# willSapgreen/structure-from-motion

Measured on AMD Instinct MI355X. Metric: BA LM-iterations/sec + final reprojection RMSE, 50 cams x 20k pts, higher is better.
Workload: dtype f64; 1 GPU; C3: 50 cams x 20000 pts/rank @ 60% visibility, lambda=5, Schur BA; observations_per_rank=599866, points_total=20000, parallelism=single GPU, collective_backend=none (plain python, no process group), collective=allreduce, schur=auto

## Files before the change

structure-from-motion_amd/csrc/sfm_ba.h:

```cpp
#pragma once

#include <utility>
#include <vector>

#include "sfm_common.h"

namespace sfm {

constexpr int kSchurCB = 18;
constexpr int kSchurRB = 128;
constexpr int kSchurMaxChunks = 128;
constexpr int kSchurKSL = 16;
constexpr int kInvRowsMaxNbk = 52;
constexpr size_t kRowsLdsBudget = 156 * 1024;
constexpr int kLinGridPerCu = 3;

constexpr int kStatSlots = 256;
constexpr int kNB = 32;
constexpr int kBlk = kNB * kNB;
__host__ __device__ inline size_t red_blk_base(int br, int bc) { return ((size_t)br * (br + 1) / 2 + bc) * kBlk; }
__host__ __device__ inline int red_blk_off(int i, int k) { return i * kNB + k; }
__host__ __device__ inline int red_lblk_off(int i, int k) { return (k >> 3) * 256 + (k & 3) * 64 + i * 2 + ((k >> 2) & 1); }
__host__ __device__ inline size_t red_index(int row, int col) {
  return red_blk_base(row >> 5, col >> 5) + red_blk_off(row & 31, col & 31);
}
__host__ __device__ inline size_t red_rhs_off(int nbk) { return (size_t)nbk * (nbk + 1) / 2 * kBlk; }
__host__ __device__ inline size_t red_size(int nbk) { return red_rhs_off(nbk) + (size_t)nbk * kNB; }

struct BaDev {
  int V = 0, N = 0;
  long long M = 0;
  int P = 0;
  int nbk = 0;
  int* pt_ptr = nullptr;
  int* cam_idx = nullptr;
  int* obs_pt = nullptr;
  double* u = nullptr;
  double* v = nullptr;
  double* cams = nullptr;
  double* px = nullptr;
  double* py = nullptr;
  double* pz = nullptr;
  CamPrep* prep[2] = {nullptr, nullptr};
  double* Z = nullptr;
  double* Zd = nullptr;
  int zp = 0;
  int zrows = 0;
  double* lin_ws = nullptr;
  double* red = nullptr;
  double* delta = nullptr;
  double* ldiag = nullptr;
  double* xinv = nullptr;
  int* sync_ctr = nullptr;
  unsigned* flow = nullptr;
  const void* flow_tasks = nullptr;
  int flow_ntasks = 0;
  int debug = 0;
  int* status = nullptr;
  int* sinfo = nullptr;
  double* cost = nullptr;
  double* cost_ws = nullptr;
  int* iter_count = nullptr;
  unsigned long long* stamps = nullptr;
};

__device__ __forceinline__ void cost_reduce(const BaDev& d, int nrows) {
  double s = 0;
  for (int r = threadIdx.x; r < nrows; r += 64) s += d.cost_ws[r];
  s = wave_sum(s);
  if (threadIdx.x == 0) d.cost[min(*d.iter_count, kStatSlots - 1)] = s;
}

__device__ __forceinline__ void cam_reduce_slice(const BaDev& d, int nrows, int t, int slice, int nslices) {
  if (t >= d.V * 35) return;
  const int per = (nrows + nslices - 1) / nslices;
  const int r0 = slice * per, r1 = min(nrows, r0 + per);
  double s = 0;
  for (int r = r0; r < r1; ++r) s += d.lin_ws[(size_t)r * d.V * 35 + t];
  if (s == 0.0) return;
  const int c = t / 35, e = t % 35;
// ... 78 lines not shown
  ~PhaseEvents() { for (hipEvent_t x : ev) (void)hipEventDestroy(x); }
  int mark(hipStream_t s) {
    if (!timed) return SFM_OK;
    hipEvent_t x;
    SFM_HIP(hipEventCreate(&x));
    ev.push_back(x);
    SFM_HIP(hipEventRecord(x, s));
    return SFM_OK;
  }
  int marks() const { return (int)ev.size(); }
  float elapsed_ms(int i) const {
    float t = 0.f;
    if (i < 0 || i + 1 >= marks() || hipEventElapsedTime(&t, ev[i], ev[i + 1]) != hipSuccess) return 0.f;
    return t;
  }
  const bool timed;
  std::vector<hipEvent_t> ev;
};

constexpr unsigned kBaMagic = 0x5F3BA001u;

struct BaScene {
  BaDev dev;
  double* own_red = nullptr;
  int max_track = 0;
  int cur = 0;
  bool prep_valid = false;
  int lin_rows = 0;
  int lin_grid = 0;
  bool red_clean = false;
  bool backsub_pending = false;
  double pending_lambda = 0;
  int pending_quirks = 0;
  bool last_reduce_deferred = false;
  bool reduce_deferred = false;
  void* schur_ws = nullptr;
  int* schur_blk_ptr = nullptr;
  bool schur_mfma_ok = false;
  const void* flow_tasks_red = nullptr;
  int flow_ntasks_red = 0;
  double* flow_camsum = nullptr;
  bool cam_list_built = false;
  int* cam_ptr = nullptr;
  int* cam_obs = nullptr;
  std::vector<int> h_cam_ptr;
  bool rows_built = false, rows_ok = false;
  void* cam_ent = nullptr;
  unsigned long long* cam_pairs = nullptr;
  std::vector<unsigned long long> h_cam_pairs;
  void* rows_table = nullptr;
  int* rows_first = nullptr;
  void* rows_ws = nullptr;
  int rows_R = 0, rows_tpr = 0, rows_wgs = 0, rows_groups = 0;
  int rows_tpl = 0, rows_cp = 7;
  std::vector<void*> owned;
};

int scene_alloc_bytes(BaScene& sc, void** ptr, size_t bytes);
template <typename T>
int scene_alloc(BaScene& sc, T*& ptr, size_t count) {
  void* q = nullptr;
  SFM_TRY(scene_alloc_bytes(sc, &q, sizeof(T) * count));
  ptr = static_cast<T*>(q);
  return SFM_OK;
}

// ... 74 lines not shown
```

structure-from-motion_amd/csrc/sfm_ba.hip:

```cpp
#include <algorithm>
#include <vector>

#include "sfm_ba.h"
#include "sfm_ba_terms.h"

namespace sfm {

__global__ void ba_cam_prep_kernel(int V, const double* __restrict__ cams, CamPrep* __restrict__ prep,
                                   int* __restrict__ status) {
  const int c = blockIdx.x * blockDim.x + threadIdx.x;
  if (c >= V) return;
  CamPrep out;
  const int st = cam_prepare(cams + 7 * c, &out);
  prep[c] = out;
  report_status(status, st, c);
}

template <int G, int LDS_MODE, bool DENSE_Z, bool FUSED, int THREADS = 256, int LOSS = SFM_LOSS_NONE>
__global__ __launch_bounds__(THREADS) void ba_linearize_kernel(BaDev d, int cur, double lambda, int quirks, LossArg<LOSS> la) {
  static_assert(!FUSED || LDS_MODE == 2, "the fused kernel keeps both camera sets in LDS");
  extern __shared__ double lds[];
  unsigned long long* stamp = (d.stamps && blockIdx.x == 0 && threadIdx.x == 0) ? d.stamps + 192 : nullptr;
  int sidx = 0;
  if (stamp) stamp[sidx++] = __builtin_amdgcn_s_memtime();
  constexpr bool PREP_LDS = LDS_MODE == 2, ACC_LDS = LDS_MODE >= 1;
  double* lds_prep = lds;
  double* lds_acc = lds + (PREP_LDS ? (size_t)d.V * 19 : 0);
  double* lds_old = lds + (size_t)d.V * (19 + 35);
  double* lds_delta = lds_old + (size_t)d.V * 19;
  const CamPrep* gprep = d.prep[cur];
  if (ACC_LDS) {
    if (PREP_LDS) {
      const double* src = reinterpret_cast<const double*>(gprep);
      for (int i = threadIdx.x; i < d.V * 19; i += blockDim.x) lds_prep[i] = src[i];
    }
    if (FUSED) {
      const double* src = reinterpret_cast<const double*>(d.prep[cur ^ 1]);
      for (int i = threadIdx.x; i < d.V * 19; i += blockDim.x) lds_old[i] = src[i];
      for (int i = threadIdx.x; i < d.V * 7; i += blockDim.x) lds_delta[i] = d.delta[i];
    }
    for (int i = threadIdx.x; i < d.V * 35; i += blockDim.x) lds_acc[i] = 0.0;
    __syncthreads();
  }
  if (FUSED) {
    const size_t n_red = red_size(d.nbk);
    for (size_t i = (size_t)blockIdx.x * blockDim.x + threadIdx.x; i < n_red; i += (size_t)gridDim.x * blockDim.x) d.red[i] = 0.0;
  }
  if (stamp) stamp[sidx++] = __builtin_amdgcn_s_memtime();
  constexpr int GPB = THREADS / G;
  const int lane_g = threadIdx.x % G;
  const int grp = threadIdx.x / G;
  double* S = d.red;
  double* rhs = d.red + red_rhs_off(d.nbk);
  double cost = 0.0;

  for (int p0 = blockIdx.x * GPB; p0 < d.N; p0 += gridDim.x * GPB) {
    const int p = p0 + grp;
    int beg = 0, end = 0;
    double X = 0, Y = 0, Z = 0;
    if (p < d.N) {
      beg = d.pt_ptr[p]; end = d.pt_ptr[p + 1];
      X = d.px[p]; Y = d.py[p]; Z = d.pz[p];
    }
    const bool single = (end - beg) <= G;
    double r[2], Jp[14], Jx[6];
    double rho = 0;
    int cam = 0;
    double uo = 0, vo = 0;
    const int o1 = beg + lane_g;
    if (single && o1 < end) { cam = d.cam_idx[o1]; uo = d.u[o1]; vo = d.v[o1]; }
    if (FUSED) {
      double a[9] = {0, 0, 0, 0, 0, 0, 0, 0, 0};
      for (int o = o1; o < end; o += G) {
        if (!single) { cam = d.cam_idx[o]; uo = d.u[o]; vo = d.v[o]; }
        CamPrep c;
        load_cam(c, reinterpret_cast<const CamPrep*>(lds_old) + cam);
        obs_terms_loss<LOSS>(c, X, Y, Z, uo, vo, quirks, la, r, Jp, Jx, rho);
        const double* dp = lds_delta + 7 * cam;
        double e0 = r[0], e1 = r[1];
#pragma unroll
        for (int i = 0; i < 7; ++i) { e0 -= Jp[i] * dp[i]; e1 -= Jp[7 + i] * dp[i]; }
        a[0] += Jx[0] * Jx[0] + Jx[3] * Jx[3];
        a[1] += Jx[1] * Jx[0] + Jx[4] * Jx[3];
        a[2] += Jx[1] * Jx[1] + Jx[4] * Jx[4];
        a[3] += Jx[2] * Jx[0] + Jx[5] * Jx[3];
        a[4] += Jx[2] * Jx[1] + Jx[5] * Jx[4];
        a[5] += Jx[2] * Jx[2] + Jx[5] * Jx[5];
        a[6] += Jx[0] * e0 + Jx[3] * e1;
        a[7] += Jx[1] * e0 + Jx[4] * e1;
        a[8] += Jx[2] * e0 + Jx[5] * e1;
      }
#pragma unroll
      for (int k = 0; k < 9; ++k) a[k] = group_sum<G>(a[k]);
      a[0] += lambda; a[2] += lambda; a[5] += lambda;
      double li[6];
      chol3_inv_fast(a, li);
      const double y0 = li[0] * a[6];
      const double y1 = li[1] * a[6] + li[2] * a[7];
      const double y2 = li[3] * a[6] + li[4] * a[7] + li[5] * a[8];
      X += li[0] * y0 + li[1] * y1 + li[3] * y2;
      Y += li[2] * y1 + li[4] * y2;
      Z += li[5] * y2;
      if (lane_g == 0 && p < d.N) { d.px[p] = X; d.py[p] = Y; d.pz[p] = Z; }
    }
    double v6[6] = {0, 0, 0, 0, 0, 0}, g3[3] = {0, 0, 0};
    for (int o = o1; o < end; o += G) {
      if (!single) { cam = d.cam_idx[o]; uo = d.u[o]; vo = d.v[o]; }
      CamPrep c;
      load_cam(c, PREP_LDS ? reinterpret_cast<const CamPrep*>(lds_prep) + cam : gprep + cam);
      obs_terms_loss<LOSS>(c, X, Y, Z, uo, vo, quirks, la, r, Jp, Jx, rho);
      v6[0] += Jx[0] * Jx[0] + Jx[3] * Jx[3];
      v6[1] += Jx[1] * Jx[0] + Jx[4] * Jx[3];
      v6[2] += Jx[1] * Jx[1] + Jx[4] * Jx[4];
      v6[3] += Jx[2] * Jx[0] + Jx[5] * Jx[3];
      v6[4] += Jx[2] * Jx[1] + Jx[5] * Jx[4];
      v6[5] += Jx[2] * Jx[2] + Jx[5] * Jx[5];
      g3[0] += Jx[0] * r[0] + Jx[3] * r[1];
      g3[1] += Jx[1] * r[0] + Jx[4] * r[1];
      g3[2] += Jx[2] * r[0] + Jx[5] * r[1];
    }
    if (stamp && sidx < 60) { asm volatile("" :: "v"(v6[0])); stamp[sidx++] = __builtin_amdgcn_s_memtime(); }
#pragma unroll
    for (int k = 0; k < 6; ++k) v6[k] = group_sum<G>(v6[k]);
#pragma unroll
    for (int k = 0; k < 3; ++k) g3[k] = group_sum<G>(g3[k]);
    v6[0] += lambda; v6[2] += lambda; v6[5] += lambda;
    double li[6];
    chol3_inv_fast(v6, li);
    const double y0 = li[0] * g3[0];
    const double y1 = li[1] * g3[0] + li[2] * g3[1];
    const double y2 = li[3] * g3[0] + li[4] * g3[1] + li[5] * g3[2];
    const double h2 = li[5] * y2;
    const double h1 = li[2] * y1 + li[4] * y2;
    const double h0 = li[0] * y0 + li[1] * y1 + li[3] * y2;
    if (stamp && sidx < 60) { asm volatile("" :: "v"(h0)); stamp[sidx++] = __builtin_amdgcn_s_memtime(); }
    for (int o = o1; o < end; o += G) {
      if (!single) {
        cam = d.cam_idx[o];
        CamPrep c;
        load_cam(c, PREP_LDS ? reinterpret_cast<const CamPrep*>(lds_prep) + cam : gprep + cam);
        obs_terms_loss<LOSS>(c, X, Y, Z, d.u[o], d.v[o], quirks, la, r, Jp, Jx, rho);
      }
      double acc[35];
      {
        double m0[3], m1[3];
        m0[0] = Jx[0] * li[0];
        m0[1] = Jx[0] * li[1] + Jx[1] * li[2];
        m0[2] = Jx[0] * li[3] + Jx[1] * li[4] + Jx[2] * li[5];
        m1[0] = Jx[3] * li[0];
        m1[1] = Jx[3] * li[1] + Jx[4] * li[2];
        m1[2] = Jx[3] * li[3] + Jx[4] * li[4] + Jx[5] * li[5];
        if (DENSE_Z) {
          double* zr = d.Zd + (size_t)(3 * p) * d.zp + 7 * cam;
          typedef double d2u __attribute__((ext_vector_type(2), aligned(8)));
#pragma unroll
          for (int j = 0; j < 3; ++j) {
            double zz[7];
#pragma unroll
            for (int i = 0; i < 7; ++i) zz[i] = Jp[i] * m0[j] + Jp[7 + i] * m1[j];
            double* row = zr + (size_t)j * d.zp;
#pragma unroll
            for (int i = 0; i < 6; i += 2) *reinterpret_cast<d2u*>(row + i) = d2u{zz[i], zz[i + 1]};
            row[6] = zz[6];
          }
        } else {
          double* zo = d.Z + (size_t)o * 21;
          typedef double d2u __attribute__((ext_vector_type(2), aligned(8)));
// ... 27 lines not shown
        for (int i = 0; i < 7; ++i) {
#pragma unroll
          for (int j = 0; j <= i; ++j) { acc[k] = Jp[i] * Jp[j] + Jp[7 + i] * Jp[7 + j]; ++k; }
          acc[28 + i] = Jp[i] * e0 + Jp[7 + i] * e1;
        }
        k = 0;
        for (int i = 0; i < 7; ++i)
          for (int j = 0; j <= i; ++j) { atomicAdd(&S[red_index(7 * cam + i, 7 * cam + j)], acc[k]); ++k; }
        for (int i = 0; i < 7; ++i) atomicAdd(&rhs[7 * cam + i], acc[28 + i]);
      }
    }
  }
  if (stamp && sidx < 62) stamp[sidx++] = __builtin_amdgcn_s_memtime();
  {
    __shared__ double wcost[THREADS / 64];
    cost = wave_sum(cost);
    if ((threadIdx.x & 63) == 0) wcost[threadIdx.x >> 6] = cost;
    __syncthreads();
    if (threadIdx.x == 0) {
      double t = 0;
#pragma unroll
      for (int w = 0; w < THREADS / 64; ++w) t += wcost[w];
      d.cost_ws[blockIdx.x] = t;
    }
  }
  if (ACC_LDS) {
    __syncthreads();
    double* row = d.lin_ws + (size_t)blockIdx.x * d.V * 35;
    for (int t = threadIdx.x; t < d.V * 35; t += blockDim.x) row[t] = lds_acc[t];
  }
  if (stamp && sidx < 63) { stamp[sidx++] = __builtin_amdgcn_s_memtime(); stamp[63] = sidx; }
}

template <int G, bool CAMS_IN_LDS, int LOSS = SFM_LOSS_NONE>
__global__ __launch_bounds__(256) void ba_backsub_kernel(BaDev d, int cur, double lambda, int quirks, LossArg<LOSS> la) {
  extern __shared__ double lds[];
  double* lds_prep = lds;
  double* lds_delta = lds + (size_t)d.V * 19;
  const CamPrep* gprep = d.prep[cur];
  if (CAMS_IN_LDS) {
    const double* src = reinterpret_cast<const double*>(gprep);
    for (int i = threadIdx.x; i < d.V * 19; i += blockDim.x) lds_prep[i] = src[i];
    for (int i = threadIdx.x; i < d.V * 7; i += blockDim.x) lds_delta[i] = d.delta[i];
    __syncthreads();
  }
  constexpr int GPB = 256 / G;
  const int lane_g = threadIdx.x % G;
  const int grp = threadIdx.x / G;
  {
    const size_t n_red = red_size(d.nbk);
    for (size_t i = (size_t)blockIdx.x * blockDim.x + threadIdx.x; i < n_red; i += (size_t)gridDim.x * blockDim.x) d.red[i] = 0.0;
  }
  for (int p0 = blockIdx.x * GPB; p0 < d.N; p0 += gridDim.x * GPB) {
    const int p = p0 + grp;
    int beg = 0, end = 0;
    double X = 0, Y = 0, Z = 0;
    if (p < d.N) {
      beg = d.pt_ptr[p]; end = d.pt_ptr[p + 1];
      X = d.px[p]; Y = d.py[p]; Z = d.pz[p];
    }
    double a[9] = {0, 0, 0, 0, 0, 0, 0, 0, 0};
    for (int o = beg + lane_g; o < end; o += G) {
      const int cam = d.cam_idx[o];
      CamPrep c;
      load_cam(c, CAMS_IN_LDS ? reinterpret_cast<const CamPrep*>(lds_prep) + cam : gprep + cam);
      double r[2], Jp[14], Jx[6], rho;
      obs_terms_loss<LOSS>(c, X, Y, Z, d.u[o], d.v[o], quirks, la, r, Jp, Jx, rho);
      const double* dp = CAMS_IN_LDS ? lds_delta + 7 * cam : d.delta + 7 * cam;
      double e0 = r[0], e1 = r[1];
#pragma unroll
      for (int i = 0; i < 7; ++i) { e0 -= Jp[i] * dp[i]; e1 -= Jp[7 + i] * dp[i]; }
      a[0] += Jx[0] * Jx[0] + Jx[3] * Jx[3];
      a[1] += Jx[1] * Jx[0] + Jx[4] * Jx[3];
      a[2] += Jx[1] * Jx[1] + Jx[4] * Jx[4];
      a[3] += Jx[2] * Jx[0] + Jx[5] * Jx[3];
      a[4] += Jx[2] * Jx[1] + Jx[5] * Jx[4];
      a[5] += Jx[2] * Jx[2] + Jx[5] * Jx[5];
      a[6] += Jx[0] * e0 + Jx[3] * e1;
      a[7] += Jx[1] * e0 + Jx[4] * e1;
      a[8] += Jx[2] * e0 + Jx[5] * e1;
    }
#pragma unroll
    for (int k = 0; k < 9; ++k) a[k] = group_sum<G>(a[k]);
    if (lane_g == 0 && p < d.N) {
      a[0] += lambda; a[2] += lambda; a[5] += lambda;
      double li[6];
      chol3_inv_fast(a, li);
      const double y0 = li[0] * a[6];
      const double y1 = li[1] * a[6] + li[2] * a[7];
      const double y2 = li[3] * a[6] + li[4] * a[7] + li[5] * a[8];
      d.px[p] = X + (li[0] * y0 + li[1] * y1 + li[3] * y2);
      d.py[p] = Y + (li[2] * y1 + li[4] * y2);
// ... 14 lines not shown
  obs_terms(c, d.px[p], d.py[p], d.pz[p], d.u[o], d.v[o], quirks, r, Jp, Jx);
  r_out[2 * o] = r[0]; r_out[2 * o + 1] = r[1];
  for (int k = 0; k < 14; ++k) Jp_out[14 * o + k] = Jp[k];
  for (int k = 0; k < 6; ++k) Jx_out[6 * o + k] = Jx[k];
}

template <int LOSS>
__global__ void ba_loss_terms_kernel(BaDev d, int cur, int quirks, LossArg<LOSS> la, double* __restrict__ s_out,
                                     double* __restrict__ w_out, double* __restrict__ rho_out) {
  const long long o = blockIdx.x * (long long)blockDim.x + threadIdx.x;
  if (o >= d.M) return;
  const int p = d.obs_pt[o];
  CamPrep c;
  load_cam(c, d.prep[cur] + d.cam_idx[o]);
  double r[2], Jp[14], Jx[6];
  obs_terms(c, d.px[p], d.py[p], d.pz[p], d.u[o], d.v[o], quirks, r, Jp, Jx);
  double s = r[0] * r[0] + r[1] * r[1], w = 1.0, sw = 1.0, rho = s;
  if constexpr (LOSS != SFM_LOSS_NONE) {
    s *= la.inv_d2;
    loss_eval<LOSS>(s, w, sw, rho);
  }
  if (s_out) s_out[o] = s;
  if (w_out) w_out[o] = w;
  if (rho_out) rho_out[o] = rho;
}

static int pick_group(const sfm_ba_problem* p) {
  double mean = p->dev.N > 0 ? (double)p->dev.M / p->dev.N : 1.0;
  int g = 4;
  while (g < 64 && g < mean) g <<= 1;
  return g;
}

template <int LDS, bool WZ, bool FUSED = false>
static void launch_linearize(const sfm_ba_problem* p, int cur, int g, int grid, size_t lds, hipStream_t s, double lambda, int quirks) {
  const BaDev& d = p->dev;
  dispatch_loss(p->loss_kind, [&](auto L) {
    constexpr int LOSS = decltype(L)::value;
    const LossArg<LOSS> la = loss_arg<LOSS>(p);
    dispatch_group<4>(g, [&](auto G) {
      if (p->deterministic)
        ba_linearize_kernel<decltype(G)::value, LDS, WZ, FUSED, 64, LOSS><<<grid, 64, lds, s>>>(d, cur, lambda, quirks, la);
      else
        ba_linearize_kernel<decltype(G)::value, LDS, WZ, FUSED, 256, LOSS><<<grid, 256, lds, s>>>(d, cur, lambda, quirks, la);
    });
  });
}

template <bool LDS>
static void launch_backsub(const sfm_ba_problem* p, int g, int grid, size_t lds, hipStream_t s, double lambda, int quirks) {
  const BaDev& d = p->dev;
  dispatch_loss(p->loss_kind, [&](auto L) {
    constexpr int LOSS = decltype(L)::value;
    const LossArg<LOSS> la = loss_arg<LOSS>(p);
    dispatch_group<4>(g, [&](auto G) {
      ba_backsub_kernel<decltype(G)::value, LDS, LOSS><<<grid, 256, lds, s>>>(d, p->cur, lambda, quirks, la);
    });
  });
}

void ba_tick(sfm_ba_problem* p, int kid, bool begin, hipStream_t s) {
  if (!(p->timing & (1 << kid))) return;
  KernelTimer& t = p->timers[kid];
  if (begin) {
    t.open = (t.calls++ % p->timing_stride) == 0;
    if (!t.open) return;
    if (t.used == (int)t.ev.size()) {
      hipEvent_t a, b;
      (void)hipEventCreate(&a); (void)hipEventCreate(&b);
      t.ev.push_back({a, b});
    }
    (void)hipEventRecord(t.ev[t.used].first, s);
  } else if (t.open) {
    (void)hipEventRecord(t.ev[t.used].second, s);
    t.used++;
    t.open = false;
  }
}

int ba_enqueue_prep(sfm_ba_problem* p) {
  hipStream_t s = p->stream;
  const BaDev& d = p->dev;
  ba_tick(p, SFM_K_PREP, true, s);
  ba_cam_prep_kernel<<<(d.V + 63) / 64, 64, 0, s>>>(d.V, d.cams, d.prep[p->cur], d.status);
  ba_tick(p, SFM_K_PREP, false, s);
  SFM_HIP(hipGetLastError());
  p->prep_valid = true;
  return SFM_OK;
}

bool ba_can_fuse(const sfm_ba_problem* p) {
  return !(p->debug & 16) && sizeof(double) * (size_t)p->dev.V * (19 + 35 + 19 + 7) <= 64 * 1024;
}

static int enqueue_backsub(sfm_ba_problem* p, double lambda, int quirks) {
  hipStream_t s = p->stream;
  const BaDev& d = p->dev;
  const int g = pick_group(p);
  const int gpb = 256 / g;
  int grid = std::min((d.N + gpb - 1) / gpb, 4 * ctx().num_cus);
  if (grid < 1) grid = 1;
  const size_t lds = sizeof(double) * (size_t)d.V * (19 + 7);
  ba_tick(p, SFM_K_BACKSUB, true, s);
  if (lds <= 64 * 1024) launch_backsub<true>(p, g, grid, lds, s, lambda, quirks);
  else launch_backsub<false>(p, g, grid, 0, s, lambda, quirks);
  ba_tick(p, SFM_K_BACKSUB, false, s);
  SFM_HIP(hipGetLastError());
  p->red_clean = true;
  p->cur ^= 1;
  return SFM_OK;
}

int ba_flush(sfm_ba_problem* p) {
  if (!p->backsub_pending) return SFM_OK;
  p->backsub_pending = false;
  return enqueue_backsub(p, p->pending_lambda, p->pending_quirks);
}

int ba_enqueue_linearize_reduce(sfm_ba_problem* p, double lambda, int quirks, bool allow_defer) {
  hipStream_t s = p->stream;
  const BaDev& d = p->dev;
  bool fused = p->backsub_pending && ba_can_fuse(p) && lambda == p->pending_lambda && quirks == p->pending_quirks;
  if (!fused) {
    SFM_TRY(ba_flush(p));
    if (!p->prep_valid) SFM_TRY(ba_enqueue_prep(p));
    if (!p->red_clean) SFM_HIP(hipMemsetAsync(d.red, 0, sizeof(double) * red_size(d.nbk), s));
  }
  p->red_clean = false;
  const int g = pick_group(p);
  const int gpb = (p->deterministic ? 64 : 256) / g;
  int grid = std::min((d.N + gpb - 1) / gpb, kLinGridPerCu * ctx().num_cus);
  if (grid < 1) grid = 1;
  const size_t lds = sizeof(double) * (size_t)d.V * (19 + 35);
  ba_tick(p, SFM_K_LINEARIZE, true, s);
  p->quirks = quirks;
  const bool dense_z = ba_schur_uses_mfma(p);
  if (dense_z) SFM_TRY(ba_schur_prepare_dense(p, s));
  if (!dense_z && d.Z == nullptr && d.M > 0) {
    SFM_TRY(scene_alloc(*p, p->dev.Z, 21 * (size_t)d.M));
  }
  const size_t lds_acc = sizeof(double) * (size_t)d.V * 35;
  const int mode = lds <= 64 * 1024 ? 2 : (lds_acc <= 64 * 1024 ? 1 : 0);
  if (fused) {
    const size_t lds_f = sizeof(double) * (size_t)d.V * (19 + 35 + 19 + 7);
    if (dense_z) launch_linearize<2, true, true>(p, p->cur ^ 1, g, grid, lds_f, s, lambda, quirks);
    else launch_linearize<2, false, true>(p, p->cur ^ 1, g, grid, lds_f, s, lambda, quirks);
    p->backsub_pending = false;
    p->cur ^= 1;
  } else if (mode == 2) {
    if (dense_z) launch_linearize<2, true>(p, p->cur, g, grid, lds, s, lambda, quirks);
    else launch_linearize<2, false>(p, p->cur, g, grid, lds, s, lambda, quirks);
  } else if (mode == 1) {
    if (dense_z) launch_linearize<1, true>(p, p->cur, g, grid, lds_acc, s, lambda, quirks);
    else launch_linearize<1, false>(p, p->cur, g, grid, lds_acc, s, lambda, quirks);
  } else {
    if (dense_z) launch_linearize<0, true>(p, p->cur, g, grid, 0, s, lambda, quirks);
    else launch_linearize<0, false>(p, p->cur, g, grid, 0, s, lambda, quirks);
  }
  p->lin_rows = mode >= 1 ? grid : 0;
  p->lin_grid = grid;
  ba_tick(p, SFM_K_LINEARIZE, false, s);
  SFM_HIP(hipGetLastError());
  SFM_TRY(ba_enqueue_schur(p, s, allow_defer));
  return SFM_OK;
}

int ba_enqueue_solve_update(sfm_ba_problem* p, double lambda, int quirks) {
  hipStream_t s = p->stream;
  SFM_TRY(ba_flush(p));
  ba_tick(p, SFM_K_SOLVE, true, s);
  SFM_TRY(ba_enqueue_reduced_solve(p, lambda));
  ba_tick(p, SFM_K_SOLVE, false, s);
  SFM_HIP(hipGetLastError());
  if (ba_can_fuse(p)) {
    p->backsub_pending = true;
    p->pending_lambda = lambda;
    p->pending_quirks = quirks;
    return SFM_OK;
  }
  return enqueue_backsub(p, lambda, quirks);
}

void ba_graph_drop(sfm_ba_problem* p) {
  for (auto& g : p->body_graph) {
    if (g) (void)hipGraphExecDestroy(g);
    g = nullptr;
  }
}

static int capture_body(sfm_ba_problem* p, double lambda, int quirks) {
  hipStream_t s = p->stream;
  const int slot = p->cur;
  SFM_HIP(hipStreamBeginCapture(s, hipStreamCaptureModeRelaxed));
  int st = ba_enqueue_linearize_reduce(p, lambda, quirks, true);
  if (st == SFM_OK) st = ba_enqueue_solve_update(p, lambda, quirks);
  hipGraph_t graph = nullptr;
  const hipError_t e = hipStreamEndCapture(s, &graph);
  if (st != SFM_OK) { if (graph) (void)hipGraphDestroy(graph); return st; }
  SFM_HIP(e);
  hipGraphExec_t exec = nullptr;
  const hipError_t ei = hipGraphInstantiate(&exec, graph, nullptr, nullptr, 0);
  (void)hipGraphDestroy(graph);
  SFM_HIP(ei);
  p->body_graph[slot] = exec;
  SFM_HIP(hipGraphLaunch(exec, s));
  return SFM_OK;
}

int ba_enqueue_iterations(sfm_ba_problem* p, double lambda, int iters, int quirks) {
  const bool graphs = p->use_graph && p->timing == 0 && p->stream != nullptr && ba_can_fuse(p) && p->comm == nullptr;
  if (graphs && (lambda != p->graph_lambda || quirks != p->graph_quirks)) {
    ba_graph_drop(p);
    p->graph_lambda = lambda;
    p->graph_quirks = quirks;
  }
  for (int it = 0; it < iters; ++it) {
    const bool steady = p->backsub_pending && lambda == p->pending_lambda && quirks == p->pending_quirks;
    if (graphs && steady) {
      if (p->body_graph[p->cur] == nullptr) {
        SFM_TRY(capture_body(p, lambda, quirks));
      } else {
        SFM_HIP(hipGraphLaunch(p->body_graph[p->cur], p->stream));
        p->cur ^= 1;
        p->red_clean = false;
        ++p->graph_replays;
      }
      continue;
    }
    SFM_TRY(ba_enqueue_linearize_reduce(p, lambda, quirks, p->comm == nullptr));
    if (p->comm) SFM_TRY(comm_all_reduce_f64(p->comm, p->dev.red, red_size(p->dev.nbk), p->stream));
    SFM_TRY(ba_enqueue_solve_update(p, lambda, quirks));
  }
  return ba_flush(p);
}

void ba_enqueue_residual_jacobian(sfm_ba_problem* p, int quirks, double* r, double* Jp, double* Jx) {
  const BaDev& d = p->dev;
  ba_residual_jacobian_kernel<<<(unsigned)((d.M + 255) / 256), 256, 0, p->stream>>>(d, p->cur, quirks, d.obs_pt, r, Jp, Jx);
}


void ba_enqueue_loss_terms(sfm_ba_problem* p, int quirks, double* s_out, double* w_out, double* rho_out) {
  const BaDev& d = p->dev;
  const unsigned grid = (unsigned)((d.M + 255) / 256);
  dispatch_loss(p->loss_kind, [&](auto L) {
    constexpr int LOSS = decltype(L)::value;
    ba_loss_terms_kernel<LOSS><<<grid, 256, 0, p->stream>>>(d, p->cur, quirks, loss_arg<LOSS>(p), s_out, w_out, rho_out);
  });
}

}
// ... 1 lines not shown
```

structure-from-motion_amd/csrc/sfm_ba_host.hip:

```cpp
#include <algorithm>
#include <vector>

#include "sfm_ba.h"
#include "sfm_ba_terms.h"
#include "sfm_scan.h"

namespace sfm {

__global__ void ba_structure_kernel(int V, int N, long long M, const int* __restrict__ pt_ptr,
                                    const int* __restrict__ cam_idx, int* __restrict__ obs_pt,
                                    int* __restrict__ blk_ptr, int nblk, int* __restrict__ sinfo) {
  const int p = blockIdx.x * blockDim.x + threadIdx.x;
  if (p >= N) return;
  const int beg = pt_ptr[p], end = pt_ptr[p + 1];
  int* row = blk_ptr + (size_t)p * (nblk + 1);
  if (beg < 0 || end < beg || end > M) {
    report_status(sinfo, 1, p);
    for (int b = 0; b <= nblk; ++b) row[b] = 0;
    return;
  }
  int prev = -1, b = 0;
  for (int o = beg; o < end; ++o) {
    const int c = cam_idx[o];
    if (c < 0 || c >= V) { report_status(sinfo, 2, o); continue; }
// ... 259 lines not shown
  SFM_HIP(hipMemcpyAsync(p->h_cam_ptr.data(), p->cam_ptr, sizeof(int) * ((size_t)V + 1), hipMemcpyDeviceToHost, s));
  SFM_TRY(stream_sync(s));
  p->cam_list_built = true;
  return SFM_OK;
}

int scene_alloc_bytes(BaScene& sc, void** ptr, size_t bytes) {
  const hipError_t e = pool_alloc(ptr, std::max<size_t>(1, bytes));
  if (e != hipSuccess) return hip_fail(e, "hipMalloc of a scene buffer", __LINE__);
  sc.owned.push_back(*ptr);
  return SFM_OK;
}

static void ba_scene_free(BaScene& sc, hipStream_t stream) {
  if (!sc.owned.empty() && ctx().inited && stream) (void)hipStreamSynchronize(stream);
  for (void* q : sc.owned) pool_free(q);
  sc = BaScene();
}

static int ba_scene_alloc(BaScene& sc, int V, int N, long long M, hipStream_t stream) {
  sc.owned.reserve(40);
  BaDev& d = sc.dev;
  d.V = V; d.N = N; d.M = M; d.P = 7 * V;
  d.nbk = (d.P + kNB - 1) / kNB;
  const size_t lin_wgs = (size_t)kLinGridPerCu * ctx().num_cus;
  SFM_TRY(scene_alloc(sc, d.pt_ptr, (size_t)N + 1));
  SFM_TRY(scene_alloc(sc, d.cam_idx, (size_t)M));
  SFM_TRY(scene_alloc(sc, d.obs_pt, (size_t)M));
  SFM_TRY(scene_alloc(sc, d.u, (size_t)M));
  SFM_TRY(scene_alloc(sc, d.v, (size_t)M));
  SFM_TRY(scene_alloc(sc, d.cams, (size_t)V * 7));
  SFM_TRY(scene_alloc(sc, d.px, (size_t)N)); SFM_TRY(scene_alloc(sc, d.py, (size_t)N)); SFM_TRY(scene_alloc(sc, d.pz, (size_t)N));
  SFM_TRY(scene_alloc(sc, d.prep[0], (size_t)V)); SFM_TRY(scene_alloc(sc, d.prep[1], (size_t)V));
  SFM_TRY(scene_alloc(sc, d.lin_ws, (sizeof(double) * V * 35 <= 64 * 1024) ? lin_wgs * V * 35 : 1));
  SFM_TRY(scene_alloc(sc, sc.own_red, red_size(d.nbk)));
  SFM_TRY(scene_alloc(sc, d.delta, (size_t)d.nbk * kNB));
  SFM_TRY(scene_alloc(sc, d.ldiag, (size_t)((d.P + 31) / 32) * 32 * 32));
  SFM_TRY(scene_alloc(sc, d.xinv, d.nbk <= kInvRowsMaxNbk ? red_rhs_off(d.nbk) : 1));
  SFM_TRY(scene_alloc(sc, d.sync_ctr, 1));
  SFM_TRY(scene_alloc(sc, d.status, 2));
  SFM_TRY(scene_alloc(sc, d.sinfo, 4));
  SFM_TRY(scene_alloc(sc, d.cost, kStatSlots));
  SFM_TRY(scene_alloc(sc, d.cost_ws, lin_wgs));
  SFM_TRY(scene_alloc(sc, d.iter_count, 1));
  d.red = sc.own_red;
  SFM_HIP(hipMemsetAsync(d.status, 0, 2 * sizeof(int), stream));
  SFM_HIP(hipMemsetAsync(d.cost, 0, kStatSlots * sizeof(double), stream));
  SFM_HIP(hipMemsetAsync(d.iter_count, 0, sizeof(int), stream));
  SFM_HIP(hipMemsetAsync(d.sync_ctr, 0, sizeof(int), stream));
  SFM_HIP(hipMemsetAsync(d.delta, 0, sizeof(double) * d.nbk * kNB, stream));
  SFM_TRY(ba_schur_plan(sc));
  return ba_flow_setup(sc, stream);
}

int ba_reset_stats(sfm_ba_problem* p) {
  SFM_HIP(hipMemsetAsync(p->dev.cost, 0, kStatSlots * sizeof(double), p->stream));
  SFM_HIP(hipMemsetAsync(p->dev.iter_count, 0, sizeof(int), p->stream));
  return SFM_OK;
}

int ba_state_changed(sfm_ba_problem* p) {
  SFM_TRY(ba_reset_stats(p));
  p->prep_valid = false;
  return SFM_OK;
}

static int ba_upload(sfm_ba_problem* p, void* dst, const void* src, size_t bytes) {
  if (bytes == 0) return SFM_OK;
  SFM_HIP(hipMemcpyAsync(dst, src, bytes, hipMemcpyHostToDevice, p->stream));
  p->upload_bytes += (long long)bytes;
  return SFM_OK;
}

static void ba_mirror_handle(sfm_ba_problem* p) {
  p->dev.debug = p->debug;
  p->dev.stamps = p->stamps;
}

static const char* ba_deterministic_obstacle(const BaScene& sc) {
  if (!sc.schur_mfma_ok) return "deterministic mode needs the dense Schur product, which does not fit this scene";
  if (sizeof(double) * (size_t)sc.dev.V * 35 > 64 * 1024) return "deterministic mode supports at most 234 cameras";
  return nullptr;
}

static int ba_adopt_grown(sfm_ba_problem* p, BaScene& sc, int n_new_cams) {
  double* const bound_red = (p->dev.red != p->own_red && n_new_cams == 0) ? p->dev.red : nullptr;
  ba_graph_drop(p);
  std::swap(static_cast<BaScene&>(*p), sc);
// ... 639 lines not shown
```

structure-from-motion_amd/csrc/sfm_ba_terms.h:

```cpp
#pragma once

#include <type_traits>

#include "sfm_ba.h"

namespace sfm {

__device__ __forceinline__ void obs_terms(const CamPrep& c, double X, double Y, double Z, double u, double v,
                                          int quirks, double* r, double* Jp, double* Jx) {
  double p[3];
  project_cam(c, X, Y, Z, 1.0, p);
  const double iz = rcp_nr(p[2]);
  jac_cam_iz(c, X, Y, Z, p, iz, quirks, Jp);
  jac_pt_cam_iz(c, p, iz, Jx);
  r[0] = u - p[0] * iz;
  r[1] = v - p[1] * iz;
}

__device__ __forceinline__ void load_cam(CamPrep& dst, const CamPrep* src) {
  const double* s = reinterpret_cast<const double*>(src);
  double* d = reinterpret_cast<double*>(&dst);
#pragma unroll
  for (int k = 0; k < 19; ++k) d[k] = s[k];
}

template <int LOSS> struct LossArg { double inv_d2, d2; };
template <> struct LossArg<SFM_LOSS_NONE> {};

template <int LOSS>
__device__ __forceinline__ void loss_eval(double s, double& w, double& sw, double& rho) {
  if (LOSS == SFM_LOSS_HUBER) {
    if (s <= 1.0) { w = 1.0; sw = 1.0; rho = s; }
    else { const double q = sqrt(s); w = 1.0 / q; sw = 1.0 / sqrt(q); rho = 2.0 * q - 1.0; }
  } else {
    const double t = 1.0 + s;
    w = 1.0 / t; sw = 1.0 / sqrt(t); rho = log1p(s);
  }
}

template <int LOSS>
__device__ __forceinline__ void obs_terms_loss(const CamPrep& c, double X, double Y, double Z, double u, double v, int quirks,
                                               const LossArg<LOSS>& la, double* r, double* Jp, double* Jx, double& rho_d2) {
  obs_terms(c, X, Y, Z, u, v, quirks, r, Jp, Jx);
  if constexpr (LOSS != SFM_LOSS_NONE) {
    double w, sw, rho;
    loss_eval<LOSS>((r[0] * r[0] + r[1] * r[1]) * la.inv_d2, w, sw, rho);
    rho_d2 = la.d2 * rho;
    r[0] *= sw; r[1] *= sw;
#pragma unroll
    for (int k = 0; k < 14; ++k) Jp[k] *= sw;
#pragma unroll
    for (int k = 0; k < 6; ++k) Jx[k] *= sw;
  }
}

template <int LOSS>
inline LossArg<LOSS> loss_arg(const sfm_ba_problem* p) {
  if constexpr (LOSS == SFM_LOSS_NONE) return {};
  else { const double d2 = p->loss_delta * p->loss_delta; return {1.0 / d2, d2}; }
}

template <class F>
inline auto dispatch_loss(int kind, F&& f) {
  switch (kind) {
    case SFM_LOSS_HUBER: return f(std::integral_constant<int, SFM_LOSS_HUBER>());
    case SFM_LOSS_CAUCHY: return f(std::integral_constant<int, SFM_LOSS_CAUCHY>());
    default: return f(std::integral_constant<int, SFM_LOSS_NONE>());
  }
}

constexpr int kCamSlice = 64;
template <class T> __host__ __device__ inline T cam_slice_count(T n) { return (n + kCamSlice - 1) / kCamSlice; }
__host__ __device__ inline size_t cam_slice_first_row(int base, int cam) { return (size_t)(base / kCamSlice) + cam; }
inline size_t cam_slice_rows(long long M, int V) { return (size_t)(M / kCamSlice) + V + 1; }

constexpr double kPtPivotTol = 1e-14;

__device__ __forceinline__ void sym3_from_li(const double* li, double* di) {
  di[0] = li[0] * li[0] + li[1] * li[1] + li[3] * li[3];
  di[1] = li[1] * li[2] + li[3] * li[4];
  di[2] = li[3] * li[5];
  di[3] = li[2] * li[2] + li[4] * li[4];
  di[4] = li[4] * li[5];
  di[5] = li[5] * li[5];
}

__device__ __forceinline__ bool sym3_finite_or_zero(bool ok, double* di) {
  ok = ok && isfinite(di[0] + di[1] + di[2] + di[3] + di[4] + di[5]);
// ... 18 lines not shown
```

structure-from-motion_amd/csrc/sfm_math.h:

```cpp
#pragma once

#include <hip/hip_runtime.h>

#include "../../include/sfm_hip.h"

#define SFM_HD __host__ __device__ __forceinline__

namespace sfm {

constexpr double kRotTol = 1e-8;
constexpr double kQwMin = 1e-6;

struct CamPrep {
  double C[3];
  double R[9];
  double t[3];
  double q[4];
};

SFM_HD void quat_to_rot(const double* q, double* R) {
  const double w = q[0], x = q[1], y = q[2], z = q[3];
  R[0] = 1 - 2 * (z * z) - 2 * (y * y);
  R[1] = -2 * z * w + 2 * y * x;
  R[2] = 2 * y * w + 2 * z * x;
// ... 79 lines not shown
  for (int i = 0; i < 3; ++i) {
    Jp[i] = (px * R[3 * i + 2] - pz * R[3 * i + 0]) * iz2;
    Jp[7 + i] = (-pz * R[3 * i + 1] - py * (sgn * R[3 * i + 2])) * iz2;
  }
  const double w2 = 2 * c.q[0], x2 = 2 * c.q[1], y2 = 2 * c.q[2], z2 = 2 * c.q[3];
  const double x4 = 4 * c.q[1], y4 = 4 * c.q[2], z4 = 4 * c.q[3];
  double A[4], B[4], C[4];
  A[0] = d1 * z2 - d2 * y2;            B[0] = d2 * x2 - d0 * z2;            C[0] = d0 * y2 - d1 * x2;
  A[1] = d1 * y2 + d2 * z2;            B[1] = d0 * y2 - d1 * x4 + d2 * w2;  C[1] = d0 * z2 - d1 * w2 - d2 * x4;
  A[2] = d1 * x2 - d0 * y4 - d2 * w2;  B[2] = d0 * x2 + d2 * z2;            C[2] = d0 * w2 + d1 * z2 - d2 * y4;
  A[3] = d1 * w2 - d0 * z4 + d2 * x2;  B[3] = d2 * y2 - d0 * w2 - d1 * z4;  C[3] = d0 * x2 + d1 * y2;
  for (int k = 0; k < 4; ++k) {
    Jp[3 + k] = (pz * A[k] - px * C[k]) * iz2;
    Jp[10 + k] = (pz * B[k] - py * C[k]) * iz2;
  }
}

SFM_HD void jac_cam_iz_urow(const CamPrep& c, double X, double Y, double Z, const double* p, double iz, double* Jp) {
  const double* R = c.R;
  const double px = p[0], pz = p[2];
  const double iz2 = iz * iz;
  const double d0 = X - c.C[0], d1 = Y - c.C[1], d2 = Z - c.C[2];
  for (int i = 0; i < 3; ++i) Jp[i] = (px * R[3 * i + 2] - pz * R[3 * i + 0]) * iz2;
  const double w2 = 2 * c.q[0], x2 = 2 * c.q[1], y2 = 2 * c.q[2], z2 = 2 * c.q[3];
  const double x4 = 4 * c.q[1], y4 = 4 * c.q[2], z4 = 4 * c.q[3];
  double A[4], C[4];
  A[0] = d1 * z2 - d2 * y2;            C[0] = d0 * y2 - d1 * x2;
  A[1] = d1 * y2 + d2 * z2;            C[1] = d0 * z2 - d1 * w2 - d2 * x4;
  A[2] = d1 * x2 - d0 * y4 - d2 * w2;  C[2] = d0 * w2 + d1 * z2 - d2 * y4;
  A[3] = d1 * w2 - d0 * z4 + d2 * x2;  C[3] = d0 * x2 + d1 * y2;
  for (int k = 0; k < 4; ++k) Jp[3 + k] = (pz * A[k] - px * C[k]) * iz2;
}

SFM_HD void jac_cam(const CamPrep& c, double X, double Y, double Z, const double* p, int quirks,
                    double* Jp) {
  jac_cam_iz(c, X, Y, Z, p, 1.0 / p[2], quirks, Jp);
}

SFM_HD void jac_pt(const double* P, const double* s, double* Jx) {
  const double iz2 = 1.0 / (s[2] * s[2]);
  for (int j = 0; j < 3; ++j) {
    Jx[j] = (s[2] * P[j] - s[0] * P[8 + j]) * iz2;
    Jx[3 + j] = (s[2] * P[4 + j] - s[1] * P[8 + j]) * iz2;
  }
}

SFM_HD void jac_pt_cam_iz(const CamPrep& c, const double* p, double iz, double* Jx) {
  const double* R = c.R;
  const double iz2 = iz * iz;
  for (int j = 0; j < 3; ++j) {
    Jx[j] = (p[2] * R[3 * j + 0] - p[0] * R[3 * j + 2]) * iz2;
    Jx[3 + j] = (p[2] * R[3 * j + 1] - p[1] * R[3 * j + 2]) * iz2;
  }
}

}
```

Measured before the change: 3926 LM-iterations/s (50cam x 20k-pt shard-iterations, all ranks).

## Carry per-point Schur factors from linearize into back substitution

The linearize kernel now stores each point's inverse Cholesky factor and step term (9 doubles) in a new carry buffer. Back substitution, both the standalone kernel and the fused next-iteration path, reuses these when lambda and quirks match. It also precomputes per-camera step maps (CamStep) in LDS, so the camera Jacobian times delta collapses to a 3x3 affine map per observation. This removes the per-point 3x3 normal-matrix rebuild and the full 14-element camera Jacobian recompute, at the cost of extra global writes and reads of 72 bytes per point and a validity-tracking state machine.

```diff
diff --git a/structure-from-motion_amd/csrc/sfm_ba.h b/structure-from-motion_amd/csrc/sfm_ba.h
--- a/structure-from-motion_amd/csrc/sfm_ba.h
+++ b/structure-from-motion_amd/csrc/sfm_ba.h
@@ -46,6 +46,7 @@
   double* Zd = nullptr;
   int zp = 0;
   int zrows = 0;
+  double* carry = nullptr;
   double* lin_ws = nullptr;
   double* red = nullptr;
   double* delta = nullptr;
@@ -190,6 +191,9 @@
   bool backsub_pending = false;
   double pending_lambda = 0;
   int pending_quirks = 0;
+  bool carry_valid = false;
+  double carry_lambda = 0;
+  int carry_quirks = 0;
   bool last_reduce_deferred = false;
   bool reduce_deferred = false;
   void* schur_ws = nullptr;
diff --git a/structure-from-motion_amd/csrc/sfm_ba.hip b/structure-from-motion_amd/csrc/sfm_ba.hip
--- a/structure-from-motion_amd/csrc/sfm_ba.hip
+++ b/structure-from-motion_amd/csrc/sfm_ba.hip
@@ -16,7 +16,7 @@
   report_status(status, st, c);
 }
 
-template <int G, int LDS_MODE, bool DENSE_Z, bool FUSED, int THREADS = 256, int LOSS = SFM_LOSS_NONE>
+template <int G, int LDS_MODE, bool DENSE_Z, int FUSED, int THREADS = 256, int LOSS = SFM_LOSS_NONE>
 __global__ __launch_bounds__(THREADS) void ba_linearize_kernel(BaDev d, int cur, double lambda, int quirks, LossArg<LOSS> la) {
   static_assert(!FUSED || LDS_MODE == 2, "the fused kernel keeps both camera sets in LDS");
   extern __shared__ double lds[];
@@ -28,13 +28,15 @@
   double* lds_acc = lds + (PREP_LDS ? (size_t)d.V * 19 : 0);
   double* lds_old = lds + (size_t)d.V * (19 + 35);
   double* lds_delta = lds_old + (size_t)d.V * 19;
+  CamStep* lds_step = reinterpret_cast<CamStep*>(lds_old);
   const CamPrep* gprep = d.prep[cur];
   if (ACC_LDS) {
+    if (FUSED == kFuseCarry) cam_steps_to_lds(d, d.prep[cur ^ 1], quirks, lds_step);
     if (PREP_LDS) {
       const double* src = reinterpret_cast<const double*>(gprep);
       for (int i = threadIdx.x; i < d.V * 19; i += blockDim.x) lds_prep[i] = src[i];
     }
-    if (FUSED) {
+    if (FUSED == kFuseRecompute) {
       const double* src = reinterpret_cast<const double*>(d.prep[cur ^ 1]);
       for (int i = threadIdx.x; i < d.V * 19; i += blockDim.x) lds_old[i] = src[i];
       for (int i = threadIdx.x; i < d.V * 7; i += blockDim.x) lds_delta[i] = d.delta[i];
@@ -69,7 +71,11 @@
     double uo = 0, vo = 0;
     const int o1 = beg + lane_g;
     if (single && o1 < end) { cam = d.cam_idx[o1]; uo = d.u[o1]; vo = d.v[o1]; }
-    if (FUSED) {
+    if (FUSED == kFuseCarry) {
+      backsub_point<G, LOSS>(d, lds_step, la, p, beg, end, lane_g, single, cam, uo, vo, X, Y, Z);
+      if (lane_g == 0 && p < d.N) { d.px[p] = X; d.py[p] = Y; d.pz[p] = Z; }
+    }
+    if (FUSED == kFuseRecompute) {
       double a[9] = {0, 0, 0, 0, 0, 0, 0, 0, 0};
       for (int o = o1; o < end; o += G) {
         if (!single) { cam = d.cam_idx[o]; uo = d.u[o]; vo = d.v[o]; }
@@ -133,6 +139,7 @@
     const double h2 = li[5] * y2;
     const double h1 = li[2] * y1 + li[4] * y2;
     const double h0 = li[0] * y0 + li[1] * y1 + li[3] * y2;
+    if (lane_g == 0 && p < d.N) carry_store(d, p, li, h0, h1, h2);
     if (stamp && sidx < 60) { asm volatile("" :: "v"(h0)); stamp[sidx++] = __builtin_amdgcn_s_memtime(); }
     for (int o = o1; o < end; o += G) {
       if (!single) {
@@ -226,13 +233,17 @@
   if (stamp && sidx < 63) { stamp[sidx++] = __builtin_amdgcn_s_memtime(); stamp[63] = sidx; }
 }
 
-template <int G, bool CAMS_IN_LDS, int LOSS = SFM_LOSS_NONE>
+template <int G, bool CAMS_IN_LDS, int LOSS = SFM_LOSS_NONE, bool CARRY = false>
 __global__ __launch_bounds__(256) void ba_backsub_kernel(BaDev d, int cur, double lambda, int quirks, LossArg<LOSS> la) {
+  static_assert(!CARRY || CAMS_IN_LDS, "the carried back substitution reads its camera steps from LDS");
   extern __shared__ double lds[];
   double* lds_prep = lds;
   double* lds_delta = lds + (size_t)d.V * 19;
   const CamPrep* gprep = d.prep[cur];
-  if (CAMS_IN_LDS) {
+  if (CARRY) {
+    cam_steps_to_lds(d, gprep, quirks, reinterpret_cast<CamStep*>(lds));
+    __syncthreads();
+  } else if (CAMS_IN_LDS) {
     const double* src = reinterpret_cast<const double*>(gprep);
     for (int i = threadIdx.x; i < d.V * 19; i += blockDim.x) lds_prep[i] = src[i];
     for (int i = threadIdx.x; i < d.V * 7; i += blockDim.x) lds_delta[i] = d.delta[i];
@@ -252,6 +263,19 @@
     if (p < d.N) {
       beg = d.pt_ptr[p]; end = d.pt_ptr[p + 1];
       X = d.px[p]; Y = d.py[p]; Z = d.pz[p];
+    }
+    if constexpr (CARRY) {
+      const bool single = (end - beg) <= G;
+      const int o1 = beg + lane_g;
+      int cam = 0;
+      double uo = 0, vo = 0;
+      if (single && o1 < end) {
+        cam = d.cam_idx[o1];
+        if (LOSS != SFM_LOSS_NONE) { uo = d.u[o1]; vo = d.v[o1]; }
+      }
+      backsub_point<G, LOSS>(d, reinterpret_cast<const CamStep*>(lds), la, p, beg, end, lane_g, single, cam, uo, vo, X, Y, Z);
+      if (lane_g == 0 && p < d.N) { d.px[p] = X; d.py[p] = Y; d.pz[p] = Z; }
+      continue;
     }
     double a[9] = {0, 0, 0, 0, 0, 0, 0, 0, 0};
     for (int o = beg + lane_g; o < end; o += G) {
@@ -332,7 +356,7 @@
   return g;
 }
 
-template <int LDS, bool WZ, bool FUSED = false>
+template <int LDS, bool WZ, int FUSED = 0>
 static void launch_linearize(const sfm_ba_problem* p, int cur, int g, int grid, size_t lds, hipStream_t s, double lambda, int quirks) {
   const BaDev& d = p->dev;
   dispatch_loss(p->loss_kind, [&](auto L) {
@@ -347,14 +371,14 @@
   });
 }
 
-template <bool LDS>
+template <bool LDS, bool CARRY = false>
 static void launch_backsub(const sfm_ba_problem* p, int g, int grid, size_t lds, hipStream_t s, double lambda, int quirks) {
   const BaDev& d = p->dev;
   dispatch_loss(p->loss_kind, [&](auto L) {
     constexpr int LOSS = decltype(L)::value;
     const LossArg<LOSS> la = loss_arg<LOSS>(p);
     dispatch_group<4>(g, [&](auto G) {
-      ba_backsub_kernel<decltype(G)::value, LDS, LOSS><<<grid, 256, lds, s>>>(d, p->cur, lambda, quirks, la);
+      ba_backsub_kernel<decltype(G)::value, LDS, LOSS, CARRY><<<grid, 256, lds, s>>>(d, p->cur, lambda, quirks, la);
     });
   });
 }
@@ -393,6 +417,10 @@
   return !(p->debug & 16) && sizeof(double) * (size_t)p->dev.V * (19 + 35 + 19 + 7) <= 64 * 1024;
 }
 
+static bool ba_carry_usable(const sfm_ba_problem* p, double lambda, int quirks) {
+  return !(p->debug & 32) && p->carry_valid && lambda == p->carry_lambda && quirks == p->carry_quirks;
+}
+
 static int enqueue_backsub(sfm_ba_problem* p, double lambda, int quirks) {
   hipStream_t s = p->stream;
   const BaDev& d = p->dev;
@@ -400,12 +428,14 @@
   const int gpb = 256 / g;
   int grid = std::min((d.N + gpb - 1) / gpb, 4 * ctx().num_cus);
   if (grid < 1) grid = 1;
-  const size_t lds = sizeof(double) * (size_t)d.V * (19 + 7);
+  const size_t lds = sizeof(double) * (size_t)d.V * (19 + 7), lds_carry = sizeof(CamStep) * (size_t)d.V;
   ba_tick(p, SFM_K_BACKSUB, true, s);
-  if (lds <= 64 * 1024) launch_backsub<true>(p, g, grid, lds, s, lambda, quirks);
+  if (ba_carry_usable(p, lambda, quirks) && lds_carry <= 64 * 1024) launch_backsub<true, true>(p, g, grid, lds_carry, s, lambda, quirks);
+  else if (lds <= 64 * 1024) launch_backsub<true>(p, g, grid, lds, s, lambda, quirks);
   else launch_backsub<false>(p, g, grid, 0, s, lambda, quirks);
   ba_tick(p, SFM_K_BACKSUB, false, s);
   SFM_HIP(hipGetLastError());
+  p->carry_valid = false;
   p->red_clean = true;
   p->cur ^= 1;
   return SFM_OK;
@@ -427,6 +457,7 @@
     if (!p->red_clean) SFM_HIP(hipMemsetAsync(d.red, 0, sizeof(double) * red_size(d.nbk), s));
   }
   p->red_clean = false;
+  const bool carry = fused && ba_carry_usable(p, lambda, quirks);
   const int g = pick_group(p);
   const int gpb = (p->deterministic ? 64 : 256) / g;
   int grid = std::min((d.N + gpb - 1) / gpb, kLinGridPerCu * ctx().num_cus);
@@ -443,8 +474,13 @@
   const int mode = lds <= 64 * 1024 ? 2 : (lds_acc <= 64 * 1024 ? 1 : 0);
   if (fused) {
     const size_t lds_f = sizeof(double) * (size_t)d.V * (19 + 35 + 19 + 7);
-    if (dense_z) launch_linearize<2, true, true>(p, p->cur ^ 1, g, grid, lds_f, s, lambda, quirks);
-    else launch_linearize<2, false, true>(p, p->cur ^ 1, g, grid, lds_f, s, lambda, quirks);
+    if (carry) {
+      if (dense_z) launch_linearize<2, true, kFuseCarry>(p, p->cur ^ 1, g, grid, lds_f, s, lambda, quirks);
+      else launch_linearize<2, false, kFuseCarry>(p, p->cur ^ 1, g, grid, lds_f, s, lambda, quirks);
+    } else {
+      if (dense_z) launch_linearize<2, true, kFuseRecompute>(p, p->cur ^ 1, g, grid, lds_f, s, lambda, quirks);
+      else launch_linearize<2, false, kFuseRecompute>(p, p->cur ^ 1, g, grid, lds_f, s, lambda, quirks);
+    }
     p->backsub_pending = false;
     p->cur ^= 1;
   } else if (mode == 2) {
@@ -459,6 +495,9 @@
   }
   p->lin_rows = mode >= 1 ? grid : 0;
   p->lin_grid = grid;
+  p->carry_valid = true;
+  p->carry_lambda = lambda;
+  p->carry_quirks = quirks;
   ba_tick(p, SFM_K_LINEARIZE, false, s);
   SFM_HIP(hipGetLastError());
   SFM_TRY(ba_enqueue_schur(p, s, allow_defer));
@@ -516,7 +555,7 @@
   }
   for (int it = 0; it < iters; ++it) {
     const bool steady = p->backsub_pending && lambda == p->pending_lambda && quirks == p->pending_quirks;
-    if (graphs && steady) {
+    if (graphs && steady && (ba_carry_usable(p, lambda, quirks) || (p->debug & 32))) {
       if (p->body_graph[p->cur] == nullptr) {
         SFM_TRY(capture_body(p, lambda, quirks));
       } else {
diff --git a/structure-from-motion_amd/csrc/sfm_ba_host.hip b/structure-from-motion_amd/csrc/sfm_ba_host.hip
--- a/structure-from-motion_amd/csrc/sfm_ba_host.hip
+++ b/structure-from-motion_amd/csrc/sfm_ba_host.hip
@@ -315,6 +315,7 @@
   SFM_TRY(scene_alloc(sc, d.cams, (size_t)V * 7));
   SFM_TRY(scene_alloc(sc, d.px, (size_t)N)); SFM_TRY(scene_alloc(sc, d.py, (size_t)N)); SFM_TRY(scene_alloc(sc, d.pz, (size_t)N));
   SFM_TRY(scene_alloc(sc, d.prep[0], (size_t)V)); SFM_TRY(scene_alloc(sc, d.prep[1], (size_t)V));
+  SFM_TRY(scene_alloc(sc, d.carry, 9 * (size_t)N));
   SFM_TRY(scene_alloc(sc, d.lin_ws, (sizeof(double) * V * 35 <= 64 * 1024) ? lin_wgs * V * 35 : 1));
   SFM_TRY(scene_alloc(sc, sc.own_red, red_size(d.nbk)));
   SFM_TRY(scene_alloc(sc, d.delta, (size_t)d.nbk * kNB));
@@ -337,6 +338,7 @@
 }
 
 int ba_reset_stats(sfm_ba_problem* p) {
+  p->carry_valid = false;
   SFM_HIP(hipMemsetAsync(p->dev.cost, 0, kStatSlots * sizeof(double), p->stream));
   SFM_HIP(hipMemsetAsync(p->dev.iter_count, 0, sizeof(int), p->stream));
   return SFM_OK;
diff --git a/structure-from-motion_amd/csrc/sfm_ba_terms.h b/structure-from-motion_amd/csrc/sfm_ba_terms.h
--- a/structure-from-motion_amd/csrc/sfm_ba_terms.h
+++ b/structure-from-motion_amd/csrc/sfm_ba_terms.h
@@ -54,6 +54,89 @@
   }
 }
 
+constexpr int kCarry = 9;
+constexpr int kFuseRecompute = 1, kFuseCarry = 2;
+
+__device__ __forceinline__ void carry_store(const BaDev& d, int p, const double* li, double h0, double h1, double h2) {
+  typedef double d2u __attribute__((ext_vector_type(2), aligned(8)));
+  double* cy = d.carry + (size_t)kCarry * p;
+  *reinterpret_cast<d2u*>(cy) = d2u{li[0], li[1]};
+  *reinterpret_cast<d2u*>(cy + 2) = d2u{li[2], li[3]};
+  *reinterpret_cast<d2u*>(cy + 4) = d2u{li[4], li[5]};
+  *reinterpret_cast<d2u*>(cy + 6) = d2u{h0, h1};
+  cy[8] = h2;
+}
+
+__device__ __forceinline__ void cam_steps_to_lds(const BaDev& d, const CamPrep* old, int quirks, CamStep* steps) {
+  for (int c = threadIdx.x; c < d.V; c += blockDim.x) {
+    CamPrep cp;
+    load_cam(cp, old + c);
+    CamStep m;
+    cam_step_map(cp, d.delta + 7 * c, quirks, &m);
+    const double* src = reinterpret_cast<const double*>(&m);
+    double* dst = reinterpret_cast<double*>(steps + c);
+#pragma unroll
+    for (int k = 0; k < 25; ++k) dst[k] = src[k];
+  }
+}
+
+template <int G, int LOSS>
+__device__ __forceinline__ void backsub_point(const BaDev& d, const CamStep* steps, const LossArg<LOSS>& la, int p, int beg,
+                                              int end, int lane_g, bool single, int cam, double uo, double vo, double& X,
+                                              double& Y, double& Z) {
+  int touch = 0;
+  if (p < d.N && lane_g < 2) touch = reinterpret_cast<const int*>(d.carry + (size_t)kCarry * p)[16 * lane_g];
+  double a[3] = {0, 0, 0};
+  for (int o = beg + lane_g; o < end; o += G) {
+    if (!single) {
+      cam = d.cam_idx[o];
+      if constexpr (LOSS != SFM_LOSS_NONE) { uo = d.u[o]; vo = d.v[o]; }
+    }
+    const CamStep* ms = steps + cam;
+    CamPrep c;
+#pragma unroll
+    for (int k = 0; k < 9; ++k) c.R[k] = ms->R[k];
+#pragma unroll
+    for (int k = 0; k < 3; ++k) c.t[k] = ms->t[k];
+    double q[3], Jx[6], s[2];
+    project_cam(c, X, Y, Z, 1.0, q);
+    const double iz = rcp_nr(q[2]);
+    jac_pt_cam_iz(c, q, iz, Jx);
+    CamStep m;
+#pragma unroll
+    for (int k = 0; k < 9; ++k) m.M[k] = ms->M[k];
+#pragma unroll
+    for (int k = 0; k < 3; ++k) m.b[k] = ms->b[k];
+    m.b2v = ms->b2v;
+    cam_step_apply(m, X, Y, Z, q, iz, s);
+    if constexpr (LOSS != SFM_LOSS_NONE) {
+      const double r0 = uo - q[0] * iz, r1 = vo - q[1] * iz;
+      double w, sw, rho;
+      loss_eval<LOSS>((r0 * r0 + r1 * r1) * la.inv_d2, w, sw, rho);
+      s[0] *= w; s[1] *= w;
+    }
+    a[0] += Jx[0] * s[0] + Jx[3] * s[1];
+    a[1] += Jx[1] * s[0] + Jx[4] * s[1];
+    a[2] += Jx[2] * s[0] + Jx[5] * s[1];
+  }
+  asm volatile("" :: "v"(touch));
+  double cy[kCarry] = {0, 0, 0, 0, 0, 0, 0, 0, 0};
+  if (p < d.N) {
+    const double* src = d.carry + (size_t)kCarry * p;
+#pragma unroll
+    for (int k = 0; k < kCarry; ++k) cy[k] = src[k];
+  }
+#pragma unroll
+  for (int k = 0; k < 3; ++k) a[k] = group_sum<G>(a[k]);
+  const double* li = cy;
+  const double y0 = li[0] * a[0];
+  const double y1 = li[1] * a[0] + li[2] * a[1];
+  const double y2 = li[3] * a[0] + li[4] * a[1] + li[5] * a[2];
+  X += cy[6] - (li[0] * y0 + li[1] * y1 + li[3] * y2);
+  Y += cy[7] - (li[2] * y1 + li[4] * y2);
+  Z += cy[8] - li[5] * y2;
+}
+
 template <int LOSS>
 inline LossArg<LOSS> loss_arg(const sfm_ba_problem* p) {
   if constexpr (LOSS == SFM_LOSS_NONE) return {};
diff --git a/structure-from-motion_amd/csrc/sfm_math.h b/structure-from-motion_amd/csrc/sfm_math.h
--- a/structure-from-motion_amd/csrc/sfm_math.h
+++ b/structure-from-motion_amd/csrc/sfm_math.h
@@ -135,6 +135,46 @@
   for (int k = 0; k < 4; ++k) Jp[3 + k] = (pz * A[k] - px * C[k]) * iz2;
 }
 
+struct CamStep {
+  double R[9];
+  double t[3];
+  double M[9];
+  double b[3];
+  double b2v;
+};
+
+SFM_HD void cam_step_map(const CamPrep& c, const double* dp, int quirks, CamStep* out) {
+  const double* R = c.R;
+  for (int i = 0; i < 9; ++i) out->R[i] = R[i];
+  for (int i = 0; i < 3; ++i) out->t[i] = c.t[i];
+  const double w2 = 2 * c.q[0], x2 = 2 * c.q[1], y2 = 2 * c.q[2], z2 = 2 * c.q[3];
+  const double x4 = 4 * c.q[1], y4 = 4 * c.q[2], z4 = 4 * c.q[3];
+  const double q0 = dp[3], q1 = dp[4], q2 = dp[5], q3 = dp[6];
+  double* M = out->M;
+  M[0] = -(y4 * q2) - z4 * q3;
+  M[1] = z2 * q0 + y2 * q1 + x2 * q2 + w2 * q3;
+  M[2] = z2 * q1 - y2 * q0 - w2 * q2 + x2 * q3;
+  M[3] = y2 * q1 - z2 * q0 + x2 * q2 - w2 * q3;
+  M[4] = -(x4 * q1) - z4 * q3;
+  M[5] = x2 * q0 + w2 * q1 + z2 * q2 + y2 * q3;
+  M[6] = y2 * q0 + z2 * q1 + w2 * q2 + x2 * q3;
+  M[7] = z2 * q2 - x2 * q0 - w2 * q1 + y2 * q3;
+  M[8] = -(x4 * q1) - y4 * q2;
+  double g[3];
+  for (int j = 0; j < 3; ++j) g[j] = R[0 + j] * dp[0] + R[3 + j] * dp[1] + R[6 + j] * dp[2];
+  for (int i = 0; i < 3; ++i) out->b[i] = -(M[3 * i] * c.C[0] + M[3 * i + 1] * c.C[1] + M[3 * i + 2] * c.C[2]) - g[i];
+  out->b2v = (quirks & SFM_Q2_LOC_JAC_SIGN) ? 2 * g[2] : 0.0;
+}
+
+SFM_HD void cam_step_apply(const CamStep& m, double X, double Y, double Z, const double* p, double iz, double* s) {
+  const double iz2 = iz * iz;
+  const double w0 = m.M[0] * X + m.M[1] * Y + m.M[2] * Z + m.b[0];
+  const double w1 = m.M[3] * X + m.M[4] * Y + m.M[5] * Z + m.b[1];
+  const double w2 = m.M[6] * X + m.M[7] * Y + m.M[8] * Z + m.b[2];
+  s[0] = (p[2] * w0 - p[0] * w2) * iz2;
+  s[1] = (p[2] * w1 - p[1] * (w2 + m.b2v)) * iz2;
+}
+
 SFM_HD void jac_cam(const CamPrep& c, double X, double Y, double Z, const double* p, int quirks,
                     double* Jp) {
   jac_cam_iz(c, X, Y, Z, p, 1.0 / p[2], quirks, Jp);
```

Measured after the change: 3918 LM-iterations/s (50cam x 20k-pt shard-iterations, all ranks), median of 3. No clear change (-0.2%).
